# kaiidams/voice100

Measured on AMD Instinct MI355X. Metric: audio frames/sec (fwd+bwd) asr_en_base, B=32x1024-frame mel, higher is better.
Workload: dtype bf16

## Files before the change

### include/voice100_hip.h

```cpp
#ifndef VOICE100_HIP_H
#define VOICE100_HIP_H

#ifdef __cplusplus
extern "C" {
#endif


int v100_dw_num_groups(int B, int C);
int v100_dwconv(const float* x, const float* x2, const float* w, const float* in_a, const float* in_b,
                const float* in_c, int in_mode, float* y, const float* aux, const float* out_a,
                const float* out_b, int out_mode, float* stats, int G, int B, int C, int Tin, int Tout,
                int K, int stride, int pad, int flip, int upsample, int force_generic, void* stream);

int v100_dwconv_wgrad(const float* g, const float* g2, const float* ga, const float* gb, const float* gc,
                      int g_mode, const float* x, const float* xa, const float* xb, int x_mode,
                      float* partial, float* dw, int G, int B, int C, int Tin, int Tout, int K, int stride,
                      int pad, int force_generic, void* stream);

int v100_dwconv_bwd(const float* g, const float* g2, const float* w, const float* ga, const float* gb,
                    const float* gc, const float* xpre, const float* xa, const float* xb, float* dxin,
                    float* stats, float* wpartial, float* dw, int G, int B, int C, int Tin, int Tout, int K,
                    int stride, int pad, int force_split, void* stream);

int v100_pw_num_parts(int B, int T);
// ... 48 lines not shown
                           void* stream);
int v100_augment_fused_len_t(const float* x, const int* len_raw, int* len_out, int* half_out, const float* uniform, float* y,
                             float* yt, int B, int Tin, int Tout, int F, int stretch_rate, float pitch_rate, float amp, int n_tmask,
                             const int* tm_s, const int* tm_e, const float* tm_a, int fm_on, int fm_s, int fm_e, float fm_a,
                             int noise_on, float noise_low, float noise_high, float noise_std, int mix, float log_offset,
                             void* stream);

int v100_shift_copy(const float* in, float* out, const float* bias, int B, int C, int Tin, int Tout, int in_ctot,
                    int in_coff, int out_ctot, int out_coff, int in_mul, int in_add, int out_mul, int out_add, int n,
                    int accumulate, void* stream);
int v100_stft_frames(const float* x, float* frames, int B, int N, int T, int hop, int win, int n_fft, void* stream);
int v100_power_spectrum(const float* spec, float* pw, int B, int F, int T, void* stream);
int v100_log_transpose(const float* in, float* out, int B, int C, int T, float offset, void* stream);
int v100_log_mel_fused(const float* x, float* out, const float* window, const float* tw256, const float* tw512, const int* mel_start,
                       const int* mel_count, const float* mel_w, int B, int N, int T, int hop, int n_fft, int n_mels, float log_offset,
                       void* stream);
int v100_world_unnormalize(const float* x, float* f0, float* logspc, float* codeap, const float* f0_mean, const float* f0_std,
                           const float* ls_mean, const float* ls_std, const float* ca_mean, const float* ca_std,
                           int B, int T, int S, int Cap, void* stream);
int v100_world_loss_parts(int B, int Tp);
int v100_world_loss(const float* pred, const float* f0, const float* hasf0, const float* logspc, const float* codeap,
                    const int* length, const float* f0_mean, const float* f0_std, const float* ls_mean, const float* ls_std,
                    const float* ca_mean, const float* ca_std, const float* w, float* partial, float* loss, float* unit,
                    int B, int Tp, int Tt, int S, int Cap, int l1, void* stream);
int v100_world_loss_bwd(const float* unit, const float* gout, float* dpred, int B, int Tp, int S, int Cap, void* stream);
int v100_exp_clip(const float* x, float* y, float offset, long long n, void* stream);

int v100_bct_to_cm(const float* in, float* out, int B, int C, int T, void* stream);
int v100_cm_to_btc(const float* in, float* out, int B, int C, int T, void* stream);

int v100_world_randn_host(float* host_out, long long n);
int v100_world_decode_aperiodicity(const float* coded, float* ap, long long rows, int nb, int fs, int fft_size, void* stream);
long long v100_world_synth_workspace_bytes(int B, int T, int fs, double frame_period_ms, int fft_size, int max_pulses);
int v100_world_synthesize(const float* f0, const float* sp, const float* ap, const float* coded_ap, int nb, const int* frames, const float* randn_table,
                          long long table_len, const float* tw256, const float* tw512, const float* dc_remover, float* y,
                          int* n_pulses, void* workspace, int B, int T, int fs, double frame_period_ms, int fft_size,
                          int max_pulses, void* stream);

int v100_im2col(const float* x, float* cols, int B, int Cin, int Tin, int Tout, int k, int stride, int pad, void* stream);
int v100_col2im(const float* dcols, float* dx, int B, int Cin, int Tin, int Tout, int k, int stride, int pad, void* stream);
int v100_pad_copy(const float* src, float* dst, int B, int C, int Tsrc, int src_step, int src_off, int n, int Tx, int lpad, void* stream);
int v100_pw_taps_supported(int B, int M, int cx, int ntap, int T, int Tx, int use_bf16);
int v100_pw_gemm_taps(const float* A, const void* A_bf16, const float* Xp, float* Y, const float* bias, const float* R,
                      int B, int M, int cx, int T, int Tx, int ntap, const int* shifts, int use_bf16, void* stream);
int v100_pw_wgrad_taps(const float* G, int Tg, int g_off, const float* Xp, float* partial, float* dW, int S, int B, int M,
                       int cx, int T, int Tx, int ntap, const int* shifts, int use_bf16, void* stream);
int v100_ln_num_parts(int B, int T);
int v100_slab_sum2(const float* partial, int parts, float* out0, float* out1, int C, void* stream);
int v100_ln_gelu_fwd(const float* y, const float* gamma, const float* beta, float eps, float* out, float* mean,
                     float* rstd, int B, int C, int T, void* stream);
int v100_ln_gelu_bwd(const float* dout, const float* y, const float* gamma, const float* beta, const float* mean,
                     const float* rstd, float* dy, float* partial, int B, int C, int T, void* stream);

long long v100_launch_count(void);
int v100_copy_probe(const void* src, void* dst, long long nbytes, void* stream);
int v100_timing_enable(int tag_mask);
int v100_timing_read(int tag, double* ms, long long* count, double* bytes);
int v100_rows_copy_probe(const void* src, void* dst, int B, int C, int row_bytes, void* stream);

int v100_pw_gemm_io(const void* A_bf16, const void* X, const void* X2, const float* xa, const float* xb, const float* xc,
                    int x_mode, void* Y, const float* ea, const float* eb, const void* R, int epi_mode, float* stats,
                    int B, int M, int K, int T, int io16, void* stream);
int v100_pw_wgrad_io(const void* G, const void* G2, const float* ga, const float* gb, const float* gc, int g_mode,
                     const void* X, const float* xa, const float* xb, int x_mode, float* partial, float* dW, int S, int B,
                     int M, int K, int T, int io16, void* stream);
int v100_dw_mfma_supported(int K, int stride);
int v100_row_pitch16(int T, int B);
int v100_dwconv_fwd_train_io(const void* a1, const float* w, const float* in_a, const float* in_b, void* a2, float* stats,
                             int G, int B, int C, int T, int K, int io16, void* stream);
int v100_dwconv_bwd_io(const void* g, const void* g2, const float* w, const float* ga, const float* gb, const float* gc,
                       const void* xpre, const float* xa, const float* xb, void* dxin, float* stats, float* wpartial,
                       float* dw, int G, int B, int C, int T, int K, int io16, void* stream);
int v100_dwconv_bwd_da1_io(const void* g, const void* g2, const float* w, const float* ga, const float* gb, const float* gc,
                           const void* xpre, const float* xa, const float* xb, void* da1_out, float* stats, float* dw,
                           const float* bn1_gamma, const float* bn1_mean, const float* bn1_rstd, float* pqr, float* dgamma,
                           float* dbeta, int B, int C, int T, int K, void* stream);
int v100_dwconv_fwd_eval_io(const void* h1, const float* w, const float* out_a, const float* out_b, void* h2, int B, int C, int T,
                            int K, int flags, void* stream);
int v100_chan_reduce2_io(const void* u, const void* v, float* partial, int G, int B, int C, int T, int io16, void* stream);
int v100_chan_affine2_shadow(const void* u, const float* v, const float* A, const float* Cc, float* out, void* shadow,
                             int B, int C, int T, int u_bf16, void* stream);
int v100_chan_affine2_io(const void* u, const void* v, const float* A, const float* Bc, const float* Cc, void* out,
                         int B, int C, int T, int io16, void* stream);
int v100_ir_act16_supported(const int* shape);

int v100_adam_chunk_elems(void);
int v100_adam_step(const void* chunks, int nchunks, const void* params, const void* grads, const void* exp_avg,
                   const void* exp_avg_sq, double lr, double beta1, double beta2, double eps, double weight_decay, int step,
                   void* stream);

int v100_grad_norm_partials(const void* chunks, int nchunks, const void* grads, void* partials, int norm_type, void* stream);
int v100_adam_step_clip(const void* chunks, int nchunks, const void* params, const void* grads, const void* exp_avg,
                        const void* exp_avg_sq, double lr, double beta1, double beta2, double eps, double weight_decay, int step,
                        int clip_mode, double clip, const void* partials, int npartials, int norm_type, void* total_norm, void* stream);
int v100_grad_clip(const void* chunks, int nchunks, const void* grads, int clip_mode, double clip, const void* partials, int npartials,
                   int norm_type, void* total_norm, void* stream);

int v100_ctc_workspace_floats(int B, int T, int Lmax);
int v100_ctc_loss_mean(const float* logits, const long long* targets, const int* in_len, const int* tgt_len, float* workspace,
                       float* nll, float* loss, float* grad, int B, int T, int V, int Lmax, int blank, void* stream);
int v100_ctc_loss(const float* logits, const long long* targets, const int* in_len, const int* tgt_len, float* workspace,
                  float* nll, float* grad, int B, int T, int V, int Lmax, int blank, void* stream);
int v100_ctc_loss_mean_t(const float* logits, const long long* targets, const int* in_len, const int* tgt_len, float* workspace,
                         float* nll, float* loss, float* grad, int grad_bvt, int B, int T, int V, int Lmax, int blank, void* stream);

long long v100_ir_prep_bytes(const int* shape);
long long v100_ir_fwd_workspace_bytes(const int* shape);
long long v100_ir_eval_cache_bytes(const int* shape);
int v100_ir_eval_prep(const int* shape, const void* const* ptrs, void* stream);
int v100_ir_fwd_eval(const int* shape, const void* const* ptrs, void* stream);
int v100_ir_stack_fwd_eval(int n, const int* shapes, const void* const* ptrs, void* stream);
int v100_ir_prep_batched(const int* shapes, const void* const* w1s, const void* const* w3s, void* const* preps, int n, void* stream);
int v100_ir_fwd_train(const int* shape, const void* const* ptrs, void* stream);
long long v100_ir_bwd_workspace_bytes(const int* shape);
int v100_ir_bwd(const int* shape, const void* const* ptrs, void* stream);

long long v100_ir_stack_plan(const int* desc, long long* plan);
int v100_ir_stack_fwd_train(const int* desc, const void* const* params, const void* x, const void* x16, void* blob, void* stream);
int v100_ir_stack_bwd(const int* desc, const void* const* params, const void* x, const void* x16, const void* blob, const void* dy,
                      void* dx, void* grads, void* ws, void* stream);

int v100_ctc_greedy_decode(const float* logits, const int* lens, long long* out, int* out_len, int B, int T, int V, int blank, void* stream);
int v100_ctc_best_path(const float* logp, const long long* labels, const int* in_len, const int* lab_len, void* back_ws, int* path,
                       float* score, int B, int T, int V, int Lmax, int max_move, void* stream);
long long v100_ctc_align_workspace_bytes(int B, int T, int Lmax);
int v100_ctc_align_block(void);
int v100_ctc_align(const float* logp, const long long* labels, const int* in_len, const int* lab_len, void* moves_ws, int* path,
                   long long* best_labels, int* align, float* score, int B, int T, int V, int Lmax, int max_move, void* stream);
int v100_align_expand(const long long* text, const double* align, const int* text_len, long long* out, int* out_len, int B, int Lmax,
                      int Tmax, int head, int tail, void* stream);


int v100_world_randn_host_f64(double* host_out, long long n);
long long v100_world_randn_bound(int kind, int T, int fs, int fft_size);
int v100_world_frames(int fs, int length, double frame_period_ms);
int v100_world_dio_bands(int fs, double f0_floor, double f0_ceil, double channels_in_octave, int* half_lengths, int max_bands);
long long v100_world_dio_workspace_bytes(int B, int max_len, int fs, double f0_floor, double f0_ceil, double channels_in_octave,
                                         double frame_period_ms);
int v100_world_dio(const float* x, const int* lengths, int B, int max_len, int pitch, int fs, double f0_floor, double f0_ceil,
                   double channels_in_octave, double frame_period_ms, double allowed_range, const double* lowcut,
                   const double* nuttall, double* f0, void* workspace, void* stream);
int v100_world_cheaptrick(const float* x, const int* lengths, const double* f0, int B, int max_len, int pitch, int fs,
                          double frame_period_ms, double q1, int fft_size, const double* randn_table, long long table_len,
                          const double* twiddle, double* sp, float* logsp, double log_offset, long long* offsets, void* stream);
long long v100_world_d4c_workspace_bytes(int B, int max_len, int fs, double frame_period_ms);
int v100_world_d4c(const float* x, const int* lengths, const double* f0, int B, int max_len, int pitch, int fs, double frame_period_ms,
                   double threshold, int fft_size, const double* randn_table, long long table_len, const double* twiddle,
                   const double* nuttall, int window_length, double* ap, double* coded, float* coded32, void* workspace, void* stream);

long long v100_lstm_weight_bytes(int H, int ndir, int use_bf16, int backward);
int v100_lstm_geometry(int H, int use_bf16, int backward, int* out);
long long v100_lstm_ws_bytes(int B, int H, int ndir, int backward);
int v100_lstm_sync_words(int B, int ndir);
int v100_lstm_persistent_ok(int B, int H, int ndir, int use_bf16, int backward);
int v100_lstm_weight_prep(const float* w_hh0, const float* w_hh1, int H, int ndir, int use_bf16, int backward, void* out,
                          void* stream);
int v100_lstm_fwd(const float* xproj, const void* w_prep, const float* b_hh0, const float* b_hh1, const int* lens, float* y,
                  float* h_n, float* c_n, float* act, float* cs, float* hprev, void* ws, unsigned* sync, int B, int T, int H,
                  int ndir, int use_bf16, int persistent, void* stream);
int v100_lstm_bwd(const float* dy, const float* dh_n, const float* dc_n, const void* w_prep, const int* lens, const float* act,
                  const float* cs, float* dgates, void* ws, unsigned* sync, int B, int T, int H, int ndir, int use_bf16,
                  int persistent, void* stream);

int v100_world_loss_v2(const float* pred, const float* f0, const float* logspc, const float* codeap, const int* length,
                       const float* f0_mean, const float* f0_std, const float* ls_mean, const float* ls_std,
                       const float* ca_mean, const float* ca_std, float* partial, float* loss, float* unit,
// ... 26 lines not shown
```

### voice100_amd/csrc/bn.hip

```cpp
#include "common.h"
#include "depthwise_common.h"
constexpr int BN_FIN_WPB = 4;

__global__ void bn_finalize_train_kernel(const float* __restrict__ stats, int parts, double count,
                                         const float* __restrict__ gamma, const float* __restrict__ beta,
                                         float* __restrict__ running_mean, float* __restrict__ running_var,
                                         long long* __restrict__ num_batches_tracked, float momentum, float eps,
                                         float* __restrict__ scale, float* __restrict__ shift,
                                         float* __restrict__ save_mean, float* __restrict__ save_rstd, int C) {
    const int c = blockIdx.x * BN_FIN_WPB + (threadIdx.x >> 6);
    const int lane = threadIdx.x & 63;
    if (c >= C) return;
    if (c == 0 && lane == 0 && num_batches_tracked) *num_batches_tracked += 1;
    double s0 = 0.0, s1 = 0.0;
    for (int g = lane; g < parts; g += 64) {
        s0 += (double)stats[((size_t)g * C + c) * 2 + 0];
        s1 += (double)stats[((size_t)g * C + c) * 2 + 1];
    }
#pragma unroll
    for (int off = 32; off > 0; off >>= 1) { s0 += __shfl_xor(s0, off, 64); s1 += __shfl_xor(s1, off, 64); }
    if (lane != 0) return;
    const double mean = s0 / count;
    double var = s1 / count - mean * mean;
    if (var < 0.0) var = 0.0;
    const float rstd = (float)(1.0 / sqrt(var + (double)eps));
    const float sc = gamma[c] * rstd;
    scale[c] = sc;
    shift[c] = beta[c] - (float)mean * sc;
    if (save_mean) save_mean[c] = (float)mean;
    if (save_rstd) save_rstd[c] = rstd;
    if (running_mean) {
        const double unbiased = count > 1.0 ? var * (count / (count - 1.0)) : var;
        running_mean[c] = (1.f - momentum) * running_mean[c] + momentum * (float)mean;
        running_var[c] = (1.f - momentum) * running_var[c] + momentum * (float)unbiased;
    }
}

__global__ void bn_eval_coeffs_kernel(const float* __restrict__ gamma, const float* __restrict__ beta,
                                      const float* __restrict__ running_mean, const float* __restrict__ running_var,
                                      float eps, float* __restrict__ scale, float* __restrict__ shift, int C) {
    const int c = blockIdx.x * blockDim.x + threadIdx.x;
    if (c >= C) return;
    const float sc = gamma[c] / sqrtf(running_var[c] + eps);
    scale[c] = sc;
    shift[c] = beta[c] - running_mean[c] * sc;
}

__global__ void bn_frozen_coeffs_kernel(const float* __restrict__ gamma, const float* __restrict__ beta,
                                        const float* __restrict__ running_mean, const float* __restrict__ running_var,
                                        float eps, float* __restrict__ scale, float* __restrict__ shift,
                                        float* __restrict__ mean, float* __restrict__ rstd, int C) {
    const int c = blockIdx.x * blockDim.x + threadIdx.x;
    if (c >= C) return;
    const float rs = 1.0f / sqrtf(running_var[c] + eps);
    const float sc = gamma[c] / sqrtf(running_var[c] + eps);
    scale[c] = sc;
    shift[c] = beta[c] - running_mean[c] * sc;
    mean[c] = running_mean[c];
    rstd[c] = rs;
}

__global__ void bn_bwd_finalize_kernel(const float* __restrict__ partial, int parts, double count,
                                       const float* __restrict__ gamma, const float* __restrict__ mean,
                                       const float* __restrict__ rstd, float* __restrict__ p, float* __restrict__ q,
                                       float* __restrict__ r, float* __restrict__ dgamma, float* __restrict__ dbeta, int C, int frozen) {
    const int c = blockIdx.x * BN_FIN_WPB + (threadIdx.x >> 6);
    const int lane = threadIdx.x & 63;
    if (c >= C) return;
    double s0 = 0.0, s1 = 0.0;
    for (int g = lane; g < parts; g += 64) {
        s0 += (double)partial[((size_t)g * C + c) * 2 + 0];
        s1 += (double)partial[((size_t)g * C + c) * 2 + 1];
    }
#pragma unroll
    for (int off = 32; off > 0; off >>= 1) { s0 += __shfl_xor(s0, off, 64); s1 += __shfl_xor(s1, off, 64); }
    if (lane != 0) return;
    const double mu = mean[c], rs = rstd[c], ga = gamma[c];
    const double dg = rs * (s1 - mu * s0);
    const double pp = ga * rs;
    const double qq = frozen ? 0.0 : -ga * rs * rs * dg / count;
    const double rr = frozen ? 0.0 : -pp * s0 / count - qq * mu;
    p[c] = (float)pp;
    q[c] = (float)qq;
    r[c] = (float)rr;
    if (dgamma) dgamma[c] = (float)dg;
    if (dbeta) dbeta[c] = (float)s0;
}

__global__ __launch_bounds__(256) void chan_reduce2_kernel(const float* __restrict__ u, const float* __restrict__ v,
                                                           float* __restrict__ partial, int B, int C, int T, int G) {
    __shared__ float red[4][2];
    const int c = blockIdx.x, g = blockIdx.y;
    const int bper = (B + G - 1) / G;
    const int b0 = g * bper, b1 = min(B, b0 + bper);
    float s0 = 0.f, s1 = 0.f;
    const bool vec = (T & 3) == 0;
    for (int b = b0; b < b1; ++b) {
        const size_t ro = ((size_t)b * C + c) * T;
        if (vec) {
            for (int t = threadIdx.x * 4; t < T; t += 1024) {
                const f32x4 a = *reinterpret_cast<const f32x4*>(u + ro + t);
                const f32x4 w = v ? *reinterpret_cast<const f32x4*>(v + ro + t) : a;
#pragma unroll
                for (int e = 0; e < 4; ++e) { s0 += a[e]; s1 = fmaf(a[e], w[e], s1); }
            }
        } else {
            for (int t = threadIdx.x; t < T; t += 256) {
                const float a = u[ro + t];
                const float w = v ? v[ro + t] : a;
                s0 += a; s1 = fmaf(a, w, s1);
            }
        }
    }
    s0 = wave_sum(s0); s1 = wave_sum(s1);
    const int lane = threadIdx.x & 63, wave = threadIdx.x >> 6;
    if (lane == 0) { red[wave][0] = s0; red[wave][1] = s1; }
    __syncthreads();
    if (threadIdx.x == 0) {
        partial[((size_t)g * C + c) * 2 + 0] = (red[0][0] + red[1][0]) + (red[2][0] + red[3][0]);
        partial[((size_t)g * C + c) * 2 + 1] = (red[0][1] + red[1][1]) + (red[2][1] + red[3][1]);
    }
}

typedef unsigned int bn_u32x2 __attribute__((ext_vector_type(2)));
template <bool B16>
__device__ __forceinline__ void chan_load4(const void* base, size_t row, int T, int P, int t, float (&o)[4]) {
    if constexpr (B16) {
        const bn_u32x2 w = *reinterpret_cast<const bn_u32x2*>(reinterpret_cast<const u16*>(base) + row * P + t);
#pragma unroll
        for (int e = 0; e < 4; ++e) {
            const unsigned d = w[e >> 1];
            o[e] = (t + e < T) ? __builtin_bit_cast(float, (e & 1) ? (d & 0xffff0000u) : (d << 16)) : 0.f;
        }
    } else {
        const float* p = reinterpret_cast<const float*>(base) + row * T + t;
        if (t + 3 < T) {
            const f32x4 v = *reinterpret_cast<const f32x4u*>(p);
#pragma unroll
            for (int e = 0; e < 4; ++e) o[e] = v[e];
        } else {
#pragma unroll
            for (int e = 0; e < 4; ++e) o[e] = (t + e < T) ? p[e] : 0.f;
        }
    }
}

template <int IO>
__global__ __launch_bounds__(256) void chan_reduce2_io_kernel(const void* __restrict__ u, const void* __restrict__ v, float* __restrict__ partial,
                                                              int B, int C, int T, int G) {
    __shared__ float red[4][2];
    const int c = blockIdx.x, g = blockIdx.y;
    const int bper = (B + G - 1) / G;
    const int b0 = g * bper, b1 = min(B, b0 + bper);
    const int P = v100_pitch16(T, B);
    float s0 = 0.f, s1 = 0.f;
    for (int b = b0; b < b1; ++b) {
        const size_t row = (size_t)b * C + c;
        for (int t = threadIdx.x * 4; t < T; t += 1024) {
            float a[4], w[4];
            chan_load4<(IO & 1) != 0>(u, row, T, P, t, a);
            chan_load4<(IO & 2) != 0>(v, row, T, P, t, w);
#pragma unroll
            for (int e = 0; e < 4; ++e) { s0 += a[e]; s1 = fmaf(a[e], w[e], s1); }
        }
    }
    s0 = wave_sum(s0); s1 = wave_sum(s1);
    const int lane = threadIdx.x & 63, wave = threadIdx.x >> 6;
    if (lane == 0) { red[wave][0] = s0; red[wave][1] = s1; }
    __syncthreads();
    if (threadIdx.x == 0) {
        partial[((size_t)g * C + c) * 2 + 0] = (red[0][0] + red[1][0]) + (red[2][0] + red[3][0]);
        partial[((size_t)g * C + c) * 2 + 1] = (red[0][1] + red[1][1]) + (red[2][1] + red[3][1]);
    }
}

template <int IO>
__global__ __launch_bounds__(1024) void chan_reduce2_fin_kernel(const void* __restrict__ u, const void* __restrict__ v, float* __restrict__ partial,
                                                                int B, int C, int T, DwFin fin) {
    __shared__ float red[16][2];
    const int c = blockIdx.x;
    const int P = v100_pitch16(T, B);
    const int T4 = (T + 3) >> 2;
    float s0 = 0.f, s1 = 0.f;
    for (int i = threadIdx.x; i < B * T4; i += 1024) {
        const int b = i / T4, t = (i - b * T4) * 4;
        const size_t row = (size_t)b * C + c;
        float a[4], w[4];
        chan_load4<(IO & 1) != 0>(u, row, T, P, t, a);
        chan_load4<(IO & 2) != 0>(v, row, T, P, t, w);
#pragma unroll
        for (int e = 0; e < 4; ++e) { s0 += a[e]; s1 = fmaf(a[e], w[e], s1); }
    }
    s0 = wave_sum(s0); s1 = wave_sum(s1);
    const int lane = threadIdx.x & 63, wave = threadIdx.x >> 6;
    if (lane == 0) { red[wave][0] = s0; red[wave][1] = s1; }
    __syncthreads();
    if (threadIdx.x == 0) {
        float t0 = 0.f, t1 = 0.f;
#pragma unroll
        for (int k = 0; k < 16; ++k) { t0 += red[k][0]; t1 += red[k][1]; }
        partial[(size_t)c * 2 + 0] = t0;
        partial[(size_t)c * 2 + 1] = t1;
        dw_finalize(fin, c, t0, t1);
    }
}

template <int NQ, bool U16 = false>
__global__ __launch_bounds__(1024) void chan_bn3_bwd_kernel(const void* __restrict__ u, const void* __restrict__ v, float* __restrict__ partial,
                                                            void* __restrict__ out, int B, int C, int T, DwFin fin) {
    __shared__ float red[16][2];
    __shared__ float coef[3];
    const int c = v100_chan_of_block<16>(blockIdx.x, C);
    const int P = v100_pitch16(T, B);
    const int T4 = (T + 3) >> 2;
    const int n = B * T4;
    float a[NQ][4], w[NQ][4];
    float s0 = 0.f, s1 = 0.f;
#pragma unroll
    for (int k = 0; k < NQ; ++k) {
        const int i = threadIdx.x + 1024 * k;
        if (i < n) {
            const int b = i / T4, t = (i - b * T4) * 4;
            const size_t row = (size_t)b * C + c;
            chan_load4<U16>(u, row, T, P, t, a[k]);
            chan_load4<true>(v, row, T, P, t, w[k]);
        } else {
#pragma unroll
            for (int e = 0; e < 4; ++e) { a[k][e] = 0.f; w[k][e] = 0.f; }
        }
    }
#pragma unroll
    for (int k = 0; k < NQ; ++k)
#pragma unroll
        for (int e = 0; e < 4; ++e) { s0 += a[k][e]; s1 = fmaf(a[k][e], w[k][e], s1); }
    s0 = wave_sum(s0); s1 = wave_sum(s1);
    const int lane = threadIdx.x & 63, wave = threadIdx.x >> 6;
    if (lane == 0) { red[wave][0] = s0; red[wave][1] = s1; }
    __syncthreads();
    if (threadIdx.x == 0) {
        float t0 = 0.f, t1 = 0.f;
#pragma unroll
        for (int k = 0; k < 16; ++k) { t0 += red[k][0]; t1 += red[k][1]; }
        partial[(size_t)c * 2 + 0] = t0;
        partial[(size_t)c * 2 + 1] = t1;
        dw_finalize_d(fin, c, (double)t0, (double)t1, coef);
    }
    __syncthreads();
    const float pa = coef[0], qb = coef[1], rc = coef[2];
#pragma unroll
    for (int k = 0; k < NQ; ++k) {
        const int i = threadIdx.x + 1024 * k;
        if (i < n) {
            const int b = i / T4, t = (i - b * T4) * 4;
            const size_t row = (size_t)b * C + c;
            float o[4];
#pragma unroll
            for (int e = 0; e < 4; ++e) o[e] = fmaf(a[k][e], pa, fmaf(w[k][e], qb, rc));
            const bn_u32x2 w16 = {pack_bf16(o[0], o[1]), pack_bf16(o[2], o[3])};
            *reinterpret_cast<bn_u32x2*>(reinterpret_cast<u16*>(out) + row * P + t) = w16;
        }
    }
}

template <int IO>
__global__ __launch_bounds__(256) void chan_affine2_io_kernel(const void* __restrict__ u, const void* __restrict__ v, const float* __restrict__ A,
                                                              const float* __restrict__ Bc, const float* __restrict__ Cc, void* __restrict__ out,
                                                              int C, int T, long rows) {
    const int P = v100_pitch16(T, (int)(rows / C));
    const int T4 = (T + 3) >> 2;
    const long total = rows * T4;
    for (long i = (long)blockIdx.x * 256 + threadIdx.x; i < total; i += (long)gridDim.x * 256) {
        const size_t row = (size_t)(i / T4);
        const int t = (int)(i % T4) * 4;
        const int c = (int)(row % C);
        const float a = A ? A[c] : 1.f, b = Bc ? Bc[c] : 1.f, cc = Cc ? Cc[c] : 0.f;
        float x[4], y[4] = {0.f, 0.f, 0.f, 0.f}, o[4];
        chan_load4<(IO & 1) != 0>(u, row, T, P, t, x);
        if (v) chan_load4<(IO & 2) != 0>(v, row, T, P, t, y);
#pragma unroll
        for (int e = 0; e < 4; ++e) o[e] = v ? fmaf(x[e], a, fmaf(y[e], b, cc)) : fmaf(x[e], a, cc);
        if constexpr ((IO & 4) != 0) {
            const bn_u32x2 w = {pack_bf16(o[0], o[1]), pack_bf16(o[2], o[3])};
            *reinterpret_cast<bn_u32x2*>(reinterpret_cast<u16*>(out) + row * P + t) = w;
        } else {
            float* q = reinterpret_cast<float*>(out) + row * T + t;
            if (t + 3 < T) { const f32x4 w = {o[0], o[1], o[2], o[3]}; *reinterpret_cast<f32x4u*>(q) = w; }
            else {
#pragma unroll
                for (int e = 0; e < 4; ++e) if (t + e < T) q[e] = o[e];
            }
        }
    }
}

template <bool UB>
__global__ __launch_bounds__(256) void chan_affine2_shadow_kernel(const void* __restrict__ u, const float* __restrict__ v, const float* __restrict__ A,
                                                                  const float* __restrict__ Cc, float* __restrict__ out, u16* __restrict__ shadow,
                                                                  int C, int T, long rows) {
    const int P = v100_pitch16(T, (int)(rows / C));
    const int T4 = (T + 3) >> 2;
    const long total = rows * T4;
    for (long i = (long)blockIdx.x * 256 + threadIdx.x; i < total; i += (long)gridDim.x * 256) {
        const size_t row = (size_t)(i / T4);
        const int t = (int)(i % T4) * 4;
        const int c = (int)(row % C);
        const float a = A ? A[c] : 1.f, cc = Cc ? Cc[c] : 0.f;
        float x[4], y[4] = {0.f, 0.f, 0.f, 0.f}, o[4];
        chan_load4<UB>(u, row, T, P, t, x);
        if (v) chan_load4<false>(v, row, T, P, t, y);
#pragma unroll
        for (int e = 0; e < 4; ++e) o[e] = v ? fmaf(x[e], a, fmaf(y[e], 1.f, cc)) : fmaf(x[e], a, cc);
        float* q = out + row * T + t;
        if (t + 3 < T) { const f32x4 w = {o[0], o[1], o[2], o[3]}; *reinterpret_cast<f32x4u*>(q) = w; }
        else {
#pragma unroll
            for (int e = 0; e < 4; ++e) if (t + e < T) q[e] = o[e];
        }
        const bn_u32x2 w16 = {pack_bf16(o[0], o[1]), pack_bf16(o[2], o[3])};
        *reinterpret_cast<bn_u32x2*>(shadow + row * P + t) = w16;
    }
}

template <bool UB, bool SH, bool VB = false>
__global__ __launch_bounds__(1024) void chan_affine2_fin_kernel(const void* __restrict__ u, const void* __restrict__ v, float* __restrict__ out,
                                                                u16* __restrict__ shadow, int B, int C, int T, DwPre pre) {
    __shared__ float coef[3];
    const int c = v100_chan_of_block<16>(blockIdx.x, C);
    if (threadIdx.x < 64) dw_finalize_parts(pre, C, c, threadIdx.x, coef);
    __syncthreads();
    const float a = coef[0], cc = coef[1];
    const int P = v100_pitch16(T, B);
    const int T4 = (T + 3) >> 2;
    for (int i = threadIdx.x; i < B * T4; i += 1024) {
        const int b = i / T4, t = (i - b * T4) * 4;
        const size_t row = (size_t)b * C + c;
        float x[4], y[4] = {0.f, 0.f, 0.f, 0.f}, o[4];
        chan_load4<UB>(u, row, T, P, t, x);
        if (v) chan_load4<VB>(v, row, T, P, t, y);
#pragma unroll
        for (int e = 0; e < 4; ++e) o[e] = v ? fmaf(x[e], a, fmaf(y[e], 1.f, cc)) : fmaf(x[e], a, cc);
        if (out) {
            float* q = out + row * T + t;
            if (t + 3 < T) { const f32x4 w = {o[0], o[1], o[2], o[3]}; *reinterpret_cast<f32x4u*>(q) = w; }
            else {
#pragma unroll
                for (int e = 0; e < 4; ++e) if (t + e < T) q[e] = o[e];
            }
        }
        if constexpr (SH) {
            const bn_u32x2 w16 = {pack_bf16(o[0], o[1]), pack_bf16(o[2], o[3])};
            *reinterpret_cast<bn_u32x2*>(shadow + row * P + t) = w16;
        }
    }
}

__global__ __launch_bounds__(256) void slab_sum0_kernel(const float* __restrict__ partial, int parts, float* __restrict__ out, int C) {
    const int c = blockIdx.x * 4 + (threadIdx.x >> 6), lane = threadIdx.x & 63;
    if (c >= C) return;
    double s = 0.0;
    for (int g = lane; g < parts; g += 64) s += (double)partial[((size_t)g * C + c) * 2];
    for (int off = 32; off > 0; off >>= 1) s += __shfl_xor(s, off, 64);
    if (lane == 0) out[c] = (float)s;
}

__global__ __launch_bounds__(256) void chan_affine2_kernel(const float* __restrict__ u, const float* __restrict__ v,
                                                           const float* __restrict__ A, const float* __restrict__ Bc,
                                                           const float* __restrict__ Cc, float* __restrict__ out,
                                                           int C, int T, long total) {
    const bool vec = (T & 3) == 0;
    if (vec) {
        const long n4 = total >> 2;
        for (long i = (long)blockIdx.x * 256 + threadIdx.x; i < n4; i += (long)gridDim.x * 256) {
            const long e0 = i << 2;
            const int c = (int)((e0 / T) % C);
            const float a = A ? A[c] : 1.f, b = Bc ? Bc[c] : 1.f, cc = Cc ? Cc[c] : 0.f;
            const f32x4 x = *reinterpret_cast<const f32x4*>(u + e0);
            f32x4 o;
            if (v) {
                const f32x4 y = *reinterpret_cast<const f32x4*>(v + e0);
#pragma unroll
                for (int e = 0; e < 4; ++e) o[e] = fmaf(x[e], a, fmaf(y[e], b, cc));
            } else {
#pragma unroll
                for (int e = 0; e < 4; ++e) o[e] = fmaf(x[e], a, cc);
            }
            *reinterpret_cast<f32x4*>(out + e0) = o;
        }
    } else {
        for (long i = (long)blockIdx.x * 256 + threadIdx.x; i < total; i += (long)gridDim.x * 256) {
            const int c = (int)((i / T) % C);
            const float a = A ? A[c] : 1.f, b = Bc ? Bc[c] : 1.f, cc = Cc ? Cc[c] : 0.f;
            out[i] = fmaf(u[i], a, (v ? v[i] * b : 0.f) + cc);
        }
    }
}

__global__ void mul_scale_kernel(const float* __restrict__ u, const float* __restrict__ m, float s, float* __restrict__ out, long n) {
    for (long i = (long)blockIdx.x * blockDim.x + threadIdx.x; i < n; i += (long)gridDim.x * blockDim.x) out[i] = u[i] * m[i] * s;
}

__device__ __forceinline__ unsigned long long splitmix64(unsigned long long z) {
    z += 0x9E3779B97F4A7C15ull;
    z = (z ^ (z >> 30)) * 0xBF58476D1CE4E5B9ull;
    z = (z ^ (z >> 27)) * 0x94D049BB133111EBull;
    return z ^ (z >> 31);
}
__global__ void dropout_fwd_kernel(const float* __restrict__ x, unsigned long long seed, unsigned thresh, float scale, float* __restrict__ y,
                                   unsigned char* __restrict__ mask, long n4, long n) {
    for (long i = (long)blockIdx.x * blockDim.x + threadIdx.x; i < n4; i += (long)gridDim.x * blockDim.x) {
        const unsigned long long r0 = splitmix64(seed ^ (unsigned long long)(2 * i) * 0xD6E8FEB86659FD93ull);
        const unsigned long long r1 = splitmix64(seed ^ (unsigned long long)(2 * i + 1) * 0xD6E8FEB86659FD93ull);
        const unsigned u[4] = {(unsigned)r0, (unsigned)(r0 >> 32), (unsigned)r1, (unsigned)(r1 >> 32)};
        const long e0 = i * 4;
        if (e0 + 3 < n) {
            const f32x4 v = *reinterpret_cast<const f32x4*>(x + e0);
            f32x4 o;
            unsigned m = 0;
#pragma unroll
            for (int e = 0; e < 4; ++e) {
                const bool keep = u[e] >= thresh;
                o[e] = keep ? v[e] * scale : 0.f;
                m |= (keep ? 1u : 0u) << (8 * e);
            }
            *reinterpret_cast<f32x4*>(y + e0) = o;
            *reinterpret_cast<unsigned*>(mask + e0) = m;
        } else {
            for (int e = 0; e < 4 && e0 + e < n; ++e) {
                const bool keep = u[e] >= thresh;
                y[e0 + e] = keep ? x[e0 + e] * scale : 0.f;
                mask[e0 + e] = keep ? 1 : 0;
            }
        }
    }
}
// ... 82 lines not shown
        const int c = c0 + ty + 8 * i, t = t0 + tx;
        if (t < T && c < C) out[((size_t)b * C + c) * T + t] = tile[tx][ty + 8 * i];
    }
}

__global__ void embedding_bwd_kernel(const long long* __restrict__ idx, const float* __restrict__ g, float* __restrict__ dtable,
                                     int V, int C, int T, long total) {
    for (long i = (long)blockIdx.x * blockDim.x + threadIdx.x; i < total; i += (long)gridDim.x * blockDim.x) {
        const int t = (int)(i % T);
        const int c = (int)((i / T) % C);
        const int b = (int)(i / ((long)T * C));
        long long id = idx[(size_t)b * T + t];
        if (id >= 0 && id < V) atomicAdd(&dtable[(size_t)id * C + c], g[i]);
    }
}

extern "C" int v100_bn_finalize_train(const float* stats, int parts, long long count, const float* gamma, const float* beta,
                                      float* running_mean, float* running_var, long long* num_batches_tracked, float momentum,
                                      float eps, float* scale, float* shift, float* save_mean, float* save_rstd, int C, void* stream) {
    if (!stats || !gamma || !beta || !scale || !shift) return V100_ERR_NULL;
    if (C <= 0 || parts <= 0 || count <= 0) return V100_ERR_SHAPE;
    V100_GGL(bn_finalize_train_kernel, dim3(ceil_div(C, BN_FIN_WPB)), dim3(64 * BN_FIN_WPB), 0, (hipStream_t)stream, stats, parts, (double)count,
                       gamma, beta, running_mean, running_var, num_batches_tracked, momentum, eps, scale, shift, save_mean, save_rstd, C);
    return v100_launch_status();
}

extern "C" int v100_bn_eval_coeffs(const float* gamma, const float* beta, const float* running_mean, const float* running_var,
                                   float eps, float* scale, float* shift, int C, void* stream) {
    if (!gamma || !beta || !running_mean || !running_var || !scale || !shift) return V100_ERR_NULL;
    if (C <= 0) return V100_ERR_SHAPE;
    V100_GGL(bn_eval_coeffs_kernel, dim3(ceil_div(C, 256)), dim3(256), 0, (hipStream_t)stream, gamma, beta, running_mean,
                       running_var, eps, scale, shift, C);
    return v100_launch_status();
}

extern "C" int v100_bn_bwd_finalize(const float* partial, int parts, long long count, const float* gamma, const float* mean,
                                    const float* rstd, float* p, float* q, float* r, float* dgamma, float* dbeta, int C, void* stream) {
    if (!partial || !gamma || !mean || !rstd || !p || !q || !r) return V100_ERR_NULL;
    if (C <= 0 || parts <= 0 || count <= 0) return V100_ERR_SHAPE;
    V100_GGL(bn_bwd_finalize_kernel, dim3(ceil_div(C, BN_FIN_WPB)), dim3(64 * BN_FIN_WPB), 0, (hipStream_t)stream, partial, parts, (double)count,
                       gamma, mean, rstd, p, q, r, dgamma, dbeta, C, 0);
    return v100_launch_status();
}

extern "C" int v100_bn_bwd_finalize_frozen(const float* partial, int parts, long long count, const float* gamma, const float* mean,
                                           const float* rstd, float* p, float* q, float* r, float* dgamma, float* dbeta, int C, void* stream) {
    if (!partial || !gamma || !mean || !rstd || !p || !q || !r) return V100_ERR_NULL;
    if (C <= 0 || parts <= 0 || count <= 0) return V100_ERR_SHAPE;
    V100_GGL(bn_bwd_finalize_kernel, dim3(ceil_div(C, BN_FIN_WPB)), dim3(64 * BN_FIN_WPB), 0, (hipStream_t)stream, partial, parts, (double)count,
                       gamma, mean, rstd, p, q, r, dgamma, dbeta, C, 1);
    return v100_launch_status();
}

extern "C" int v100_bn_frozen_coeffs(const float* gamma, const float* beta, const float* running_mean, const float* running_var,
                                     float eps, float* scale, float* shift, float* mean, float* rstd, int C, void* stream) {
    if (!gamma || !beta || !running_mean || !running_var || !scale || !shift || !mean || !rstd) return V100_ERR_NULL;
    if (C <= 0) return V100_ERR_SHAPE;
    V100_GGL(bn_frozen_coeffs_kernel, dim3(ceil_div(C, 256)), dim3(256), 0, (hipStream_t)stream, gamma, beta, running_mean,
                       running_var, eps, scale, shift, mean, rstd, C);
    return v100_launch_status();
}

extern "C" int v100_chan_reduce2(const float* u, const float* v, float* partial, int G, int B, int C, int T, void* stream) {
    if (!u || !partial) return V100_ERR_NULL;
    if (B <= 0 || C <= 0 || T <= 0 || G <= 0 || G > B) return V100_ERR_SHAPE;
    V100_GGL(chan_reduce2_kernel, dim3(C, G), dim3(256), 0, (hipStream_t)stream, u, v, partial, B, C, T, G);
    return v100_launch_status();
}

extern "C" int v100_chan_reduce2_io(const void* u, const void* v, float* partial, int G, int B, int C, int T, int io16, void* stream) {
    if (!u || !v || !partial) return V100_ERR_NULL;
    if (B <= 0 || C <= 0 || T <= 0 || G <= 0 || G > B) return V100_ERR_SHAPE;
    if (io16 == 2) V100_GGL(chan_reduce2_io_kernel<2>, dim3(C, G), dim3(256), 0, (hipStream_t)stream, u, v, partial, B, C, T, G);
    else return V100_ERR_SHAPE;
    return v100_launch_status();
}

int chan_affine2_fin(const void* u, const void* v, float* out, void* shadow, int B, int C, int T, int u_bf16, const DwPre& pre, void* stream,
                     int v_bf16) {
    if (!u || (!out && !shadow) || !pre.stats) return V100_ERR_NULL;
    if (B <= 0 || C <= 0 || T <= 0 || pre.f.mode != 1 || pre.parts <= 0) return V100_ERR_SHAPE;
    if (v_bf16 && !u_bf16) return V100_ERR_SHAPE;
    hipStream_t st = (hipStream_t)stream;
#define CAF(UB_, SH_, VB_) V100_GGL((chan_affine2_fin_kernel<UB_, SH_, VB_>), dim3(C), dim3(1024), 0, st, u, v, out, (u16*)shadow, B, C, T, pre)
    if (v_bf16) { if (shadow) CAF(true, true, true); else CAF(true, false, true); }
    else if (u_bf16) { if (shadow) CAF(true, true, false); else CAF(true, false, false); }
    else { if (shadow) CAF(false, true, false); else CAF(false, false, false); }
#undef CAF
    return v100_launch_status();
}

int chan_bn3_bwd_fits(int B, int T) { return (long)B * ((T + 3) / 4) <= 1024 * 8; }
int chan_bn3_bwd(const void* u, const void* v, float* partial, void* out, int B, int C, int T, const DwFin& fin, void* stream, int u_bf16) {
    if (!u || !v || !partial || !out || fin.mode != 2) return 0;
    const long n = (long)B * ((T + 3) / 4);
    hipStream_t st = (hipStream_t)stream;
#define CB3(NQ_) do { if (u_bf16) V100_GGL((chan_bn3_bwd_kernel<NQ_, true>), dim3(C), dim3(1024), 0, st, u, v, partial, out, B, C, T, fin); \
                      else V100_GGL((chan_bn3_bwd_kernel<NQ_, false>), dim3(C), dim3(1024), 0, st, u, v, partial, out, B, C, T, fin); } while (0)
    if (n <= 1024 * 2) CB3(2);
    else if (n <= 1024 * 4) CB3(4);
    else if (n <= 1024 * 6) CB3(6);
    else if (n <= 1024 * 8) CB3(8);
    else return 0;
#undef CB3
    return 1;
}

int chan_reduce2_io_fin(const void* u, const void* v, float* partial, int B, int C, int T, const DwFin& fin, void* stream) {
    if (!u || !v || !partial) return V100_ERR_NULL;
    if (B <= 0 || C <= 0 || T <= 0 || fin.mode != 2) return V100_ERR_SHAPE;
    V100_GGL(chan_reduce2_fin_kernel<2>, dim3(C), dim3(1024), 0, (hipStream_t)stream, u, v, partial, B, C, T, fin);
    return v100_launch_status();
}

extern "C" int v100_chan_affine2_io(const void* u, const void* v, const float* A, const float* Bc, const float* Cc, void* out,
                                    int B, int C, int T, int io16, void* stream) {
    if (!u || !out) return V100_ERR_NULL;
    if (B <= 0 || C <= 0 || T <= 0) return V100_ERR_SHAPE;
    const long rows = (long)B * C;
    const long total = rows * ((T + 3) / 4);
    long blocks = (total + 255) / 256;
    if (blocks > 4096) blocks = 4096;
    if (blocks < 1) blocks = 1;
    hipStream_t st = (hipStream_t)stream;
    if (io16 == 1) V100_GGL(chan_affine2_io_kernel<1>, dim3((unsigned)blocks), dim3(256), 0, st, u, v, A, Bc, Cc, out, C, T, rows);
    else if (io16 == 6) V100_GGL(chan_affine2_io_kernel<6>, dim3((unsigned)blocks), dim3(256), 0, st, u, v, A, Bc, Cc, out, C, T, rows);
    else return V100_ERR_SHAPE;
    return v100_launch_status();
}

extern "C" int v100_chan_affine2_shadow(const void* u, const float* v, const float* A, const float* Cc, float* out, void* shadow,
                                        int B, int C, int T, int u_bf16, void* stream) {
    if (!u || !out || !shadow) return V100_ERR_NULL;
    if (B <= 0 || C <= 0 || T <= 0) return V100_ERR_SHAPE;
    const long rows = (long)B * C;
    const long total = rows * ((T + 3) / 4);
    long blocks = (total + 255) / 256;
    if (blocks > 4096) blocks = 4096;
    if (blocks < 1) blocks = 1;
    hipStream_t st = (hipStream_t)stream;
    if (u_bf16) V100_GGL(chan_affine2_shadow_kernel<true>, dim3((unsigned)blocks), dim3(256), 0, st, u, v, A, Cc, out, (u16*)shadow, C, T, rows);
    else V100_GGL(chan_affine2_shadow_kernel<false>, dim3((unsigned)blocks), dim3(256), 0, st, u, v, A, Cc, out, (u16*)shadow, C, T, rows);
    return v100_launch_status();
}

extern "C" int v100_slab_sum0(const float* partial, int parts, float* out, int C, void* stream) {
    if (!partial || !out) return V100_ERR_NULL;
    if (parts <= 0 || C <= 0) return V100_ERR_SHAPE;
    V100_GGL(slab_sum0_kernel, dim3(ceil_div(C, 4)), dim3(256), 0, (hipStream_t)stream, partial, parts, out, C);
    return v100_launch_status();
}

extern "C" int v100_chan_affine2(const float* u, const float* v, const float* A, const float* Bc, const float* Cc, float* out,
                                 int B, int C, int T, void* stream) {
    if (!u || !out) return V100_ERR_NULL;
    if (B <= 0 || C <= 0 || T <= 0) return V100_ERR_SHAPE;
    const long total = (long)B * C * T;
    long blocks = (total / 4 + 255) / 256;
    if (blocks > 4096) blocks = 4096;
    if (blocks < 1) blocks = 1;
    V100_GGL(chan_affine2_kernel, dim3((unsigned)blocks), dim3(256), 0, (hipStream_t)stream, u, v, A, Bc, Cc, out, C, T, total);
    return v100_launch_status();
}

extern "C" int v100_mul_scale(const float* u, const float* m, float s, float* out, long long n, void* stream) {
    if (!u || !m || !out) return V100_ERR_NULL;
    if (n <= 0) return V100_ERR_SHAPE;
    long blocks = (n + 255) / 256;
    if (blocks > 4096) blocks = 4096;
    V100_GGL(mul_scale_kernel, dim3((unsigned)blocks), dim3(256), 0, (hipStream_t)stream, u, m, s, out, (long)n);
    return v100_launch_status();
}

extern "C" int v100_dropout_fwd(const float* x, long long seed, float p, float* y, void* mask, long long n, void* stream) {
    if (!x || !y || !mask) return V100_ERR_NULL;
    if (n <= 0 || !(p >= 0.f && p < 1.f)) return V100_ERR_SHAPE;
    const long n4 = (n + 3) / 4;
    long blocks = (n4 + 255) / 256;
    if (blocks > 4096) blocks = 4096;
    const double t = (double)p * 4294967296.0;
    const unsigned thresh = t >= 4294967295.0 ? 4294967295u : (unsigned)t;
    V100_GGL(dropout_fwd_kernel, dim3((unsigned)blocks), dim3(256), 0, (hipStream_t)stream, x, (unsigned long long)seed, thresh,
                       1.0f / (1.0f - p), y, (unsigned char*)mask, n4, (long)n);
    return v100_launch_status();
}

extern "C" int v100_dropout_bwd(const float* dy, const void* mask, float p, float* dx, long long n, void* stream) {
    if (!dy || !dx || !mask) return V100_ERR_NULL;
    if (n <= 0 || !(p >= 0.f && p < 1.f)) return V100_ERR_SHAPE;
    const long n4 = (n + 3) / 4;
    long blocks = (n4 + 255) / 256;
    if (blocks > 4096) blocks = 4096;
    V100_GGL(dropout_bwd_kernel, dim3((unsigned)blocks), dim3(256), 0, (hipStream_t)stream, dy, (const unsigned char*)mask,
                       1.0f / (1.0f - p), dx, n4, (long)n);
// ... 47 lines not shown
```

Measured before the change: 10.07 million.

## Prefetch channel tiles with buffer loads before BN finalize in fused kernels

Changes the fused BN forward-affine and backward kernels so that every thread issues all of its register-resident input loads (raw buffer loads, with out-of-range lanes sent to an OOB offset) before wave 0 finalizes the BN statistics. The global-memory latency of the data loads then overlaps the stats reduction and the barrier, instead of starting only after the coefficients are ready. The BN parameters are preloaded and pinned in scalar registers. The change also adds C entry points for the fused kernels and size guards against the buffer-descriptor range. In exchange it uses more registers and adds more template instantiations.

Result: no change. 10.12 million (median of 6 runs) (+0.5%).

```diff
diff --git a/include/voice100_hip.h b/include/voice100_hip.h
--- a/include/voice100_hip.h
+++ b/include/voice100_hip.h
@@ -154,6 +154,13 @@
                              int B, int C, int T, int u_bf16, void* stream);
 int v100_chan_affine2_io(const void* u, const void* v, const float* A, const float* Bc, const float* Cc, void* out,
                          int B, int C, int T, int io16, void* stream);
+int v100_chan_affine2_fin_io(const void* u, const void* v, float* out, void* shadow, const float* stats, int parts, const float* gamma,
+                             const float* beta, float* running_mean, float* running_var, long long* num_batches_tracked,
+                             float momentum, float eps, float* scale, float* shift, float* save_mean, float* save_rstd,
+                             int B, int C, int T, int io16, void* stream);
+int v100_chan_bn3_bwd_io(const void* u, const void* v, float* partial, void* out, const float* gamma, const float* mean,
+                         const float* rstd, float* p, float* q, float* r, float* dgamma, float* dbeta, int B, int C, int T,
+                         int io16, void* stream);
 int v100_ir_act16_supported(const int* shape);
 
 int v100_adam_chunk_elems(void);
diff --git a/voice100_amd/csrc/bn.hip b/voice100_amd/csrc/bn.hip
--- a/voice100_amd/csrc/bn.hip
+++ b/voice100_amd/csrc/bn.hip
@@ -1,4 +1,5 @@
 #include "common.h"
+#include "../../include/voice100_hip.h"
 #include "depthwise_common.h"
 constexpr int BN_FIN_WPB = 4;
 
@@ -123,15 +124,27 @@
 }
 
 typedef unsigned int bn_u32x2 __attribute__((ext_vector_type(2)));
+template <bool B16> struct ChanQuad { typedef bn_u32x2 type; };
+template <> struct ChanQuad<false> { typedef f32x4 type; };
+template <bool B16>
+__device__ __forceinline__ void chan_decode4(const typename ChanQuad<B16>::type& w, int t, int T, float (&o)[4]) {
+#pragma unroll
+    for (int e = 0; e < 4; ++e) {
+        float val;
+        if constexpr (B16) {
+            const unsigned d = w[e >> 1];
+            val = __builtin_bit_cast(float, (e & 1) ? (d & 0xffff0000u) : (d << 16));
+        } else {
+            val = w[e];
+        }
+        o[e] = (t + e < T) ? val : 0.f;
+    }
+}
 template <bool B16>
 __device__ __forceinline__ void chan_load4(const void* base, size_t row, int T, int P, int t, float (&o)[4]) {
     if constexpr (B16) {
         const bn_u32x2 w = *reinterpret_cast<const bn_u32x2*>(reinterpret_cast<const u16*>(base) + row * P + t);
-#pragma unroll
-        for (int e = 0; e < 4; ++e) {
-            const unsigned d = w[e >> 1];
-            o[e] = (t + e < T) ? __builtin_bit_cast(float, (e & 1) ? (d & 0xffff0000u) : (d << 16)) : 0.f;
-        }
+        chan_decode4<true>(w, t, T, o);
     } else {
         const float* p = reinterpret_cast<const float*>(base) + row * T + t;
         if (t + 3 < T) {
@@ -174,6 +187,21 @@
     }
 }
 
+constexpr int CHAN_OOB = 0x7ffffff0;
+constexpr size_t CHAN_BUF_MAX = 0x7ffffff0;
+template <bool B16>
+__device__ __forceinline__ typename ChanQuad<B16>::type chan_issue4(__amdgpu_buffer_rsrc_t rs, int voff) {
+    if constexpr (B16) return __builtin_bit_cast(bn_u32x2, __builtin_amdgcn_raw_buffer_load_b64(rs, voff, 0, 0));
+    else return __builtin_bit_cast(f32x4, __builtin_amdgcn_raw_buffer_load_b128(rs, voff, 0, 0));
+}
+template <bool B16>
+__device__ __forceinline__ int chan_quad_off(int row, int T, int P, int t) {
+    return B16 ? (row * P + t) * 2 : (row * T + t) * 4;
+}
+static inline size_t chan_tensor_bytes(bool b16, int B, int C, int T) {
+    return (size_t)B * C * (b16 ? (size_t)v100_pitch16(T, B) * 2 : (size_t)T * 4);
+}
+
 template <int IO>
 __global__ __launch_bounds__(1024) void chan_reduce2_fin_kernel(const void* __restrict__ u, const void* __restrict__ v, float* __restrict__ partial,
                                                                 int B, int C, int T, DwFin fin) {
@@ -214,20 +242,29 @@
     const int P = v100_pitch16(T, B);
     const int T4 = (T + 3) >> 2;
     const int n = B * T4;
+    float fmu = fin.a[c], frs = fin.b[c], fga = fin.gamma[c];
+    const __amdgpu_buffer_rsrc_t ru = dw_make_rsrc(u, (unsigned)((size_t)B * C * (U16 ? (size_t)P * 2 : (size_t)T * 4)));
+    const __amdgpu_buffer_rsrc_t rv = dw_make_rsrc(v, (unsigned)((size_t)B * C * P * 2));
+    typename ChanQuad<U16>::type ua[NQ];
+    bn_u32x2 va[NQ];
+    int tq[NQ], oq[NQ];
+#pragma unroll
+    for (int k = 0; k < NQ; ++k) {
+        const int i = threadIdx.x + 1024 * k;
+        const int b = i / T4, row = b * C + c;
+        tq[k] = (i - b * T4) * 4;
+        oq[k] = i < n ? chan_quad_off<true>(row, T, P, tq[k]) : CHAN_OOB;
+        ua[k] = chan_issue4<U16>(ru, i < n ? chan_quad_off<U16>(row, T, P, tq[k]) : CHAN_OOB);
+        va[k] = chan_issue4<true>(rv, oq[k]);
+    }
+    __builtin_amdgcn_sched_barrier(0);
+    asm volatile("" : "+s"(fmu), "+s"(frs), "+s"(fga));
     float a[NQ][4], w[NQ][4];
     float s0 = 0.f, s1 = 0.f;
 #pragma unroll
     for (int k = 0; k < NQ; ++k) {
-        const int i = threadIdx.x + 1024 * k;
-        if (i < n) {
-            const int b = i / T4, t = (i - b * T4) * 4;
-            const size_t row = (size_t)b * C + c;
-            chan_load4<U16>(u, row, T, P, t, a[k]);
-            chan_load4<true>(v, row, T, P, t, w[k]);
-        } else {
-#pragma unroll
-            for (int e = 0; e < 4; ++e) { a[k][e] = 0.f; w[k][e] = 0.f; }
-        }
+        chan_decode4<U16>(ua[k], tq[k], T, a[k]);
+        chan_decode4<true>(va[k], tq[k], T, w[k]);
     }
 #pragma unroll
     for (int k = 0; k < NQ; ++k)
@@ -243,22 +280,18 @@
         for (int k = 0; k < 16; ++k) { t0 += red[k][0]; t1 += red[k][1]; }
         partial[(size_t)c * 2 + 0] = t0;
         partial[(size_t)c * 2 + 1] = t1;
-        dw_finalize_d(fin, c, (double)t0, (double)t1, coef);
+        dw_finalize_bwd_pre(fin, c, (double)t0, (double)t1, fmu, frs, fga, coef);
     }
     __syncthreads();
     const float pa = coef[0], qb = coef[1], rc = coef[2];
+    const __amdgpu_buffer_rsrc_t ro = dw_make_rsrc(out, (unsigned)((size_t)B * C * P * 2));
 #pragma unroll
     for (int k = 0; k < NQ; ++k) {
-        const int i = threadIdx.x + 1024 * k;
-        if (i < n) {
-            const int b = i / T4, t = (i - b * T4) * 4;
-            const size_t row = (size_t)b * C + c;
-            float o[4];
-#pragma unroll
-            for (int e = 0; e < 4; ++e) o[e] = fmaf(a[k][e], pa, fmaf(w[k][e], qb, rc));
-            const bn_u32x2 w16 = {pack_bf16(o[0], o[1]), pack_bf16(o[2], o[3])};
-            *reinterpret_cast<bn_u32x2*>(reinterpret_cast<u16*>(out) + row * P + t) = w16;
-        }
+        float o[4];
+#pragma unroll
+        for (int e = 0; e < 4; ++e) o[e] = fmaf(a[k][e], pa, fmaf(w[k][e], qb, rc));
+        const bn_u32x2 w16 = {pack_bf16(o[0], o[1]), pack_bf16(o[2], o[3])};
+        __builtin_amdgcn_raw_buffer_store_b64(w16, ro, oq[k], 0, 0);
     }
 }
 
@@ -321,22 +354,46 @@
     }
 }
 
-template <bool UB, bool SH, bool VB = false>
+__device__ __forceinline__ void chan_pre_finish_fwd(const DwPre& pre, int c, int lane, const DwPreRegs& r, float* coef) {
+#pragma clang fp contract(off)
+    double s0 = 0.0, s1 = 0.0;
+#pragma unroll
+    for (int i = 0; i < 4; ++i) { s0 += (double)r.s[i][0]; s1 += (double)r.s[i][1]; }
+#pragma unroll
+    for (int off = 32; off > 0; off >>= 1) { s0 += __shfl_xor(s0, off, 64); s1 += __shfl_xor(s1, off, 64); }
+    if (lane != 0) return;
+    const DwFin& f = pre.f;
+    if (c == 0 && f.num_batches_tracked) *f.num_batches_tracked += 1;
+    const double mean = s0 / f.count;
+    double var = __builtin_fma(-mean, mean, s1 / f.count);
+    if (var < 0.0) var = 0.0;
+    const float rstd = (float)(1.0 / sqrt(var + (double)f.eps));
+    const float sc = r.ga * rstd;
+    const float sh = __builtin_fmaf(-sc, (float)mean, r.a);
+    f.o0[c] = sc;
+    f.o1[c] = sh;
+    if (f.o3) f.o3[c] = (float)mean;
+    if (f.o4) f.o4[c] = rstd;
+    if (f.running_mean) {
+        const double unbiased = f.count > 1.0 ? var * (f.count / (f.count - 1.0)) : var;
+        const float keep = 1.f - f.momentum;
+        f.running_mean[c] = __builtin_fmaf(f.momentum, (float)mean, keep * r.rm);
+        f.running_var[c] = __builtin_fmaf(keep, r.rv, f.momentum * (float)unbiased);
+    }
+    coef[0] = sc; coef[1] = sh; coef[2] = 0.f;
+}
+
+template <bool UB, bool SH, bool VB, int NQ>
 __global__ __launch_bounds__(1024) void chan_affine2_fin_kernel(const void* __restrict__ u, const void* __restrict__ v, float* __restrict__ out,
                                                                 u16* __restrict__ shadow, int B, int C, int T, DwPre pre) {
     __shared__ float coef[3];
     const int c = v100_chan_of_block<16>(blockIdx.x, C);
-    if (threadIdx.x < 64) dw_finalize_parts(pre, C, c, threadIdx.x, coef);
-    __syncthreads();
-    const float a = coef[0], cc = coef[1];
     const int P = v100_pitch16(T, B);
     const int T4 = (T + 3) >> 2;
-    for (int i = threadIdx.x; i < B * T4; i += 1024) {
-        const int b = i / T4, t = (i - b * T4) * 4;
+    const int n = B * T4;
+    auto emit = [&](int b, int t, const float (&x)[4], const float (&y)[4], float a, float cc) {
         const size_t row = (size_t)b * C + c;
-        float x[4], y[4] = {0.f, 0.f, 0.f, 0.f}, o[4];
-        chan_load4<UB>(u, row, T, P, t, x);
-        if (v) chan_load4<VB>(v, row, T, P, t, y);
+        float o[4];
 #pragma unroll
         for (int e = 0; e < 4; ++e) o[e] = v ? fmaf(x[e], a, fmaf(y[e], 1.f, cc)) : fmaf(x[e], a, cc);
         if (out) {
@@ -350,6 +407,51 @@
         if constexpr (SH) {
             const bn_u32x2 w16 = {pack_bf16(o[0], o[1]), pack_bf16(o[2], o[3])};
             *reinterpret_cast<bn_u32x2*>(shadow + row * P + t) = w16;
+        }
+    };
+    if constexpr (NQ == 0) {
+        if (threadIdx.x < 64) dw_finalize_parts(pre, C, c, threadIdx.x, coef);
+        __syncthreads();
+        const float a = coef[0], cc = coef[1];
+        for (int i = threadIdx.x; i < n; i += 1024) {
+            const int b = i / T4, t = (i - b * T4) * 4;
+            const size_t row = (size_t)b * C + c;
+            float x[4], y[4] = {0.f, 0.f, 0.f, 0.f};
+            chan_load4<UB>(u, row, T, P, t, x);
+            if (v) chan_load4<VB>(v, row, T, P, t, y);
+            emit(b, t, x, y, a, cc);
+        }
+    } else {
+        const int lane = threadIdx.x & 63;
+        const bool wave0 = __builtin_amdgcn_readfirstlane((int)threadIdx.x >> 6) == 0;
+        DwPreRegs prer;
+        dw_pre_issue(pre, C, c, lane, wave0, pre.stats, prer);
+        const __amdgpu_buffer_rsrc_t ru = dw_make_rsrc(u, (unsigned)((size_t)B * C * (UB ? (size_t)P * 2 : (size_t)T * 4)));
+        const __amdgpu_buffer_rsrc_t rv = dw_make_rsrc(v ? v : u, v ? (unsigned)((size_t)B * C * (VB ? (size_t)P * 2 : (size_t)T * 4)) : 0u);
+        typename ChanQuad<UB>::type xr[NQ];
+        typename ChanQuad<VB>::type yr[NQ];
+        int bq[NQ], tq[NQ];
+#pragma unroll
+        for (int k = 0; k < NQ; ++k) {
+            const int i = threadIdx.x + 1024 * k;
+            bq[k] = i / T4;
+            tq[k] = (i - bq[k] * T4) * 4;
+            const int row = bq[k] * C + c;
+            xr[k] = chan_issue4<UB>(ru, i < n ? chan_quad_off<UB>(row, T, P, tq[k]) : CHAN_OOB);
+            yr[k] = chan_issue4<VB>(rv, i < n ? chan_quad_off<VB>(row, T, P, tq[k]) : CHAN_OOB);
+        }
+        __builtin_amdgcn_sched_barrier(0);
+        if (wave0) chan_pre_finish_fwd(pre, c, lane, prer, coef);
+        __syncthreads();
+        const float a = coef[0], cc = coef[1];
+#pragma unroll
+        for (int k = 0; k < NQ; ++k) {
+            if ((int)threadIdx.x + 1024 * k < n) {
+                float x[4], y[4];
+                chan_decode4<UB>(xr[k], tq[k], T, x);
+                chan_decode4<VB>(yr[k], tq[k], T, y);
+                emit(bq[k], tq[k], x, y, a, cc);
+            }
         }
     }
 }
@@ -598,11 +700,18 @@
     if (B <= 0 || C <= 0 || T <= 0 || pre.f.mode != 1 || pre.parts <= 0) return V100_ERR_SHAPE;
     if (v_bf16 && !u_bf16) return V100_ERR_SHAPE;
     hipStream_t st = (hipStream_t)stream;
-#define CAF(UB_, SH_, VB_) V100_GGL((chan_affine2_fin_kernel<UB_, SH_, VB_>), dim3(C), dim3(1024), 0, st, u, v, out, (u16*)shadow, B, C, T, pre)
+    const long n = (long)B * ((T + 3) / 4);
+    int nq = n <= 1024 * 2 ? 2 : n <= 1024 * 4 ? 4 : n <= 1024 * 6 ? 6 : n <= 1024 * 8 ? 8 : 0;
+    if (pre.parts > DW_PRE_MAXPARTS || (size_t)pre.parts * C * 8 > CHAN_BUF_MAX || chan_tensor_bytes(u_bf16 != 0, B, C, T) > CHAN_BUF_MAX ||
+        (v && chan_tensor_bytes(v_bf16 != 0, B, C, T) > CHAN_BUF_MAX)) nq = 0;
+#define CAF_(UB_, SH_, VB_, NQ_) V100_GGL((chan_affine2_fin_kernel<UB_, SH_, VB_, NQ_>), dim3(C), dim3(1024), 0, st, u, v, out, (u16*)shadow, B, C, T, pre)
+#define CAF(UB_, SH_, VB_) do { if (nq == 2) CAF_(UB_, SH_, VB_, 2); else if (nq == 4) CAF_(UB_, SH_, VB_, 4); else if (nq == 6) CAF_(UB_, SH_, VB_, 6); \
+                                else if (nq == 8) CAF_(UB_, SH_, VB_, 8); else CAF_(UB_, SH_, VB_, 0); } while (0)
     if (v_bf16) { if (shadow) CAF(true, true, true); else CAF(true, false, true); }
     else if (u_bf16) { if (shadow) CAF(true, true, false); else CAF(true, false, false); }
     else { if (shadow) CAF(false, true, false); else CAF(false, false, false); }
 #undef CAF
+#undef CAF_
     return v100_launch_status();
 }
 
@@ -610,6 +719,7 @@
 int chan_bn3_bwd(const void* u, const void* v, float* partial, void* out, int B, int C, int T, const DwFin& fin, void* stream, int u_bf16) {
     if (!u || !v || !partial || !out || fin.mode != 2) return 0;
     const long n = (long)B * ((T + 3) / 4);
+    if (chan_tensor_bytes(u_bf16 != 0, B, C, T) > CHAN_BUF_MAX || chan_tensor_bytes(true, B, C, T) > CHAN_BUF_MAX) return 0;
     hipStream_t st = (hipStream_t)stream;
 #define CB3(NQ_) do { if (u_bf16) V100_GGL((chan_bn3_bwd_kernel<NQ_, true>), dim3(C), dim3(1024), 0, st, u, v, partial, out, B, C, T, fin); \
                       else V100_GGL((chan_bn3_bwd_kernel<NQ_, false>), dim3(C), dim3(1024), 0, st, u, v, partial, out, B, C, T, fin); } while (0)
@@ -626,6 +736,27 @@
     if (!u || !v || !partial) return V100_ERR_NULL;
     if (B <= 0 || C <= 0 || T <= 0 || fin.mode != 2) return V100_ERR_SHAPE;
     V100_GGL(chan_reduce2_fin_kernel<2>, dim3(C), dim3(1024), 0, (hipStream_t)stream, u, v, partial, B, C, T, fin);
+    return v100_launch_status();
+}
+
+extern "C" int v100_chan_affine2_fin_io(const void* u, const void* v, float* out, void* shadow, const float* stats, int parts, const float* gamma,
+                                        const float* beta, float* running_mean, float* running_var, long long* num_batches_tracked,
+                                        float momentum, float eps, float* scale, float* shift, float* save_mean, float* save_rstd,
+                                        int B, int C, int T, int io16, void* stream) {
+    if (!stats || !gamma || !beta || !scale || !shift) return V100_ERR_NULL;
+    if (B <= 0 || C <= 0 || T <= 0 || (io16 & ~3)) return V100_ERR_SHAPE;
+    const DwPre pre{{1, (double)B * T, gamma, beta, nullptr, scale, shift, nullptr, save_mean, save_rstd, running_mean, running_var,
+                     num_batches_tracked, momentum, eps}, stats, parts};
+    return chan_affine2_fin(u, v, out, shadow, B, C, T, io16 & 1, pre, stream, (io16 & 2) ? 1 : 0);
+}
+
+extern "C" int v100_chan_bn3_bwd_io(const void* u, const void* v, float* partial, void* out, const float* gamma, const float* mean,
+                                    const float* rstd, float* p, float* q, float* r, float* dgamma, float* dbeta, int B, int C, int T,
+                                    int io16, void* stream) {
+    if (!u || !v || !partial || !out || !gamma || !mean || !rstd || !p || !q || !r) return V100_ERR_NULL;
+    if (B <= 0 || C <= 0 || T <= 0 || (io16 & ~1)) return V100_ERR_SHAPE;
+    const DwFin fin{2, (double)B * T, gamma, mean, rstd, p, q, r, dgamma, dbeta, nullptr, nullptr, nullptr, 0.f, 0.f};
+    if (!chan_bn3_bwd(u, v, partial, out, B, C, T, fin, stream, io16 & 1)) return V100_ERR_SHAPE;
     return v100_launch_status();
 }
 
```
